# HannesStark/3DInfomax

Hardware: AMD Instinct MI355X
Metric: molecules/sec pretraining step (PNA+Net3D, QM9-50k); PNA-agg HBM GB/s vs peak (higher is better)
Workload: dtype f32

## Files before the change

### 3dinfomax_amd/net3d_native.py

```python
import ctypes
import os

import torch

from . import _lib, ops, tape
from .layer_native import _Arena, _al, _tail
from .layers import _composite_ok, _keeps_pre, _set_workspaces

NATIVE_NET3D = True
BF16_STORE = True
BF16_STORE_MIN_EDGES = 1 << 20
FUSED_EDGE = True
_F32 = torch.float32


def _chk(rc, name):
    if rc != 0:
        _lib.check(rc, name)


def _blocks(model):
    b = model.__dict__.get('_i3d_blocks')
    if b is None:
        layers = [(list(l.message_network.fully_connected), l.soft_edge_network, list(l.update_network.fully_connected), l.reduce_mean)
                  for l in model.mp_layers]
        nw = list(model.node_wise_output_network.fully_connected) if model.node_wise_output_layers > 0 else []
        b = model.__dict__['_i3d_blocks'] = (model.edge_input.fully_connected[0], layers, nw, list(model.output.fully_connected))
    return b


def eligible(model, g):
    if not (NATIVE_NET3D and model.training and not model.use_node_features):
        return False
    idx = g.index()
    if g.device.type != 'cuda' or idx.num_edges == 0 or idx.num_graphs == 0:
        return False
    edge_in, layers, nw, out = _blocks(model)
    fcs = [edge_in] + [fc for m, _, u, _ in layers for fc in m + u] + nw + out[:-1]
    for fc in fcs:
        h = fc.hot()
        if not (_composite_ok(h[4]) and h[0].is_cuda and h[0].is_contiguous() and h[1] is not None and fc.bias):
            return False
    last = out[-1].hot()
    if last[4].bn is not None:
        if not (_composite_ok(last[4]) and last[0].is_contiguous()):
            return False
    elif last[4].act is not None or not last[0].is_contiguous() or last[1] is None:
        return False
    return len(layers) >= 1 and all(len(m) >= 1 and len(u) >= 1 for m, _, u, _ in layers)


def fused_edge_ok(model):
    ok = model.__dict__.get('_i3d_fused_edge')
    if ok is None:
        edge_in, layers, nw, out = _blocks(model)
        ok = False
        if len(layers) == 1 and len(layers[0][0]) == 1:
            H = model.node_embedding.shape[0]
            w_in, spec_in = edge_in.hot('silu')[0], edge_in.hot('silu')[4]
            w_m, spec_m = layers[0][0][0].hot()[0], layers[0][0][0].hot()[4]
            n_enc = model.fourier_encodings
            din = 2 * n_enc + 1 if n_enc > 0 else 1
            ok = (tuple(w_in.shape) == (H, din) and tuple(w_m.shape) == (H, 3 * H) and spec_in.act == 'silu'
                  and spec_m.act == 'silu' and spec_m.post_act is None
                  and bool(_lib.load().i3d_net3d_edge_supported(H, n_enc)))
        model.__dict__['_i3d_fused_edge'] = ok
    return ok and FUSED_EDGE


def _edge_stage_fwd(L, stream, ar, dev, model, g, idx, d_raw, edge_in, msg_fc, se, reduce_mean, N, E, H):
    a = _lib.Net3dEdgeArgs()
    W_in, b_in, g_in, be_in, spec_in = edge_in.hot('silu')[:5]
    W_m, b_m, g_m, be_m, spec_m = msg_fc.hot()[:5]
    _tail(a.tail_in, spec_in, g_in, be_in, ar.take(H), ar.take(H), H, dev)
    _tail(a.tail_msg, spec_m, g_m, be_m, ar.take(H), ar.take(H), H, dev)
    a.num_nodes, a.num_edges, a.hidden, a.n_enc, a.reduce_mean = N, E, H, model.fourier_encodings, int(reduce_mean)
    a.ld_w_in, a.ld_w_msg = W_in.stride(0), W_m.stride(0)
    a.d_raw, a.perm, a.dst_s, a.in_ptr = d_raw.data_ptr(), idx.perm.data_ptr(), idx.dst_s.data_ptr(), idx.in_ptr.data_ptr()
    a.emb = model.node_embedding.data_ptr()
    a.W_in, a.b_in, a.W_msg, a.b_msg = W_in.data_ptr(), b_in.data_ptr(), W_m.data_ptr(), b_m.data_ptr()
    a.w_gate, a.b_gate = se.weight.data_ptr(), se.bias.data_ptr()
    a.stats = ar.take(int(L.i3d_net3d_edge_stats_floats(E, H)))
    a.aff_in, a.aff_msg = ar.take(3 * H), ar.take(3 * H)
    a.x_msg, a.msg, a.m_sum = ar.take(E * H), ar.take(E * H), ar.take(N * H)
    d_out = torch.empty(E, H, dtype=_F32, device=dev)
    a.d_out = d_out.data_ptr()
    a.store_bf16 = int(BF16_STORE and E >= BF16_STORE_MIN_EDGES and L.i3d_get_matmul_precision() != 0)
    a.x_center = ar.take(H)
    _chk(L.i3d_net3d_edge_fwd(ctypes.byref(a), stream), 'i3d_net3d_edge_fwd')
    return a, a.m_sum, d_out, (W_in, b_in, g_in, be_in, W_m, b_m, g_m, be_m, se.weight, se.bias)


class _Rec:
    __slots__ = ('kind', 'a', 'fc', 'rows', 'fin', 'fout', 'x', 'y', 'extra')

    def __init__(self, kind, **kw):
        self.a = self.fc = self.extra = None
        self.rows = self.fin = self.fout = self.x = self.y = 0
        self.kind = kind
        for k, v in kw.items():
            setattr(self, k, v)


def _fc_floats(rows, fout, spec):
    return _al(rows * fout) * (3 if _keeps_pre(spec) else 2) + 2 * _al(fout)


def _fc_fwd(L, stream, ar, dev, fc, rows, x_ptr, residual=None, post_act=None, y_ptr=None):
    W, b, gamma, beta, spec = fc.hot(post_act)[:5]
    fout, fin = W.shape
    a = _lib.FcArgs()
    _tail(a.tail, spec, gamma, beta, ar.take(fout), ar.take(fout), fout, dev)
    a.rows, a.f_in, a.f_out, a.ldw = rows, fin, fout, W.stride(0)
    a.x, a.W, a.bias, a.residual = x_ptr, W.data_ptr(), b.data_ptr(), residual
    a.xact = ar.take(rows * fout)
    a.pre_keep = ar.take(rows * fout) if _keeps_pre(spec) else None
    a.y = y_ptr if y_ptr is not None else ar.take(rows * fout)
    _chk(L.i3d_fc_bn_fwd(ctypes.byref(a), stream), 'i3d_fc_bn_fwd')
    return _Rec('fc', a=a, fc=fc, rows=rows, fin=fin, fout=fout, x=x_ptr, y=a.y, extra=(W, b, gamma, beta, residual is not None))


def forward(ctx, model, g, params):
    idx = g.index()
    dev = g.device
    N, E, B = idx.num_nodes, idx.num_edges, idx.num_graphs
    edge_in, layers, nw, out = _blocks(model)
    H = model.node_embedding.shape[0]
    n_enc = model.fourier_encodings
    enc_dim = 2 * n_enc + 1 if n_enc > 0 else 1
    codes = model._readout_codes
    R = len(codes)
    L = _lib.load()
    stream = ops._stream()

    fused = fused_edge_ok(model)
    total = _al(N * H)
    if fused:
        total += 5 * _al(H) + 2 * _al(3 * H) + _al(int(L.i3d_net3d_edge_stats_floats(E, H))) + 2 * _al(E * H) + 2 * _al(N * H)
    else:
        total += _al(E) + (_al(E * enc_dim) if n_enc > 0 else 0) + _fc_floats(E, H, edge_in.hot('silu')[4])
    for msg, se, upd, _ in layers:
        if not fused:
            Fo = msg[0].hot()[0].shape[0]
            total += _al(N * 2 * Fo) + _al(E * Fo) + _fc_floats(E, Fo, msg[0].hot()[4])
            for fc in msg[1:]:
                total += _fc_floats(E, fc.hot()[0].shape[0], fc.hot()[4])
            total += _al(E * H) * 2 + _al(E) + _al(N * H) * 2
        for fc in upd:
            total += _fc_floats(N, fc.hot()[0].shape[0], fc.hot()[4])
    for fc in nw:
        total += _fc_floats(N, fc.hot()[0].shape[0], fc.hot()[4])
    total += _al(B * R * H)
    for fc in out:
        total += _fc_floats(B, fc.hot()[0].shape[0], fc.hot()[4]) if fc.hot()[4].bn is not None else 0
    ar = _Arena(total + 64, dev)
    tr = {'layers': [], 'nw': [], 'out': []}

    d_raw = g.edata['d']
    if d_raw.dtype != _F32 or not d_raw.is_contiguous():
        d_raw = d_raw.contiguous().float()
    emb = model.node_embedding
    h = ar.take(N * H)
    _chk(L.i3d_broadcast_row(emb.data_ptr(), N, H, h, stream), 'i3d_broadcast_row')
    d_out = d = None
    if not fused:
        dperm = ar.take(E)
        _chk(L.i3d_gather_rows(d_raw.data_ptr(), idx.perm.data_ptr(), E, 1, dperm, stream), 'i3d_gather_rows')
        enc = dperm
        if n_enc > 0:
            enc = ar.take(E * enc_dim)
            _chk(L.i3d_fourier_encode(dperm, E, n_enc, enc, stream), 'i3d_fourier_encode')
        tr['edge_in'] = _fc_fwd(L, stream, ar, dev, edge_in, E, enc, post_act='silu')
        d = tr['edge_in'].y

    last_h_fc = nw[-1] if nw else layers[-1][2][-1]
    h_out = torch.empty(N, last_h_fc.hot()[0].shape[0], dtype=_F32, device=dev)
    n_layers = len(layers)
    for li, (msg, se, upd, reduce_mean) in enumerate(layers):
        last_layer = li + 1 == n_layers
        lay = {'msg': [], 'upd': []}
        if fused:
            lay['fused'], m_sum, d_out, ctx.fused_params = _edge_stage_fwd(L, stream, ar, dev, model, g, idx, d_raw, edge_in,
                                                                           msg[0], se, reduce_mean, N, E, H)
            u = ar.take(N * H)
            _chk(L.i3d_add(m_sum, h, N * H, u, stream), 'i3d_add')
            x = u
            for k, fc in enumerate(upd):
                final = k + 1 == len(upd)
                y_ptr = h_out.data_ptr() if (final and not nw) else None
                r = _fc_fwd(L, stream, ar, dev, fc, N, x, residual=h if final else None, y_ptr=y_ptr)
                lay['upd'].append(r)
                x = r.y
            tr['layers'].append(lay)
            h = x
            break
        W, b, gamma, beta, spec = msg[0].hot()[:5]
        Fo = W.shape[0]
        a = _lib.EdgeFcArgs()
        _tail(a.tail, spec, gamma, beta, ar.take(Fo), ar.take(Fo), Fo, dev)
        a.num_nodes, a.num_edges, a.f_h, a.f_q, a.f_out, a.ldw = N, E, H, H, Fo, W.stride(0)
        a.h, a.q, a.W, a.bias = h, d, W.data_ptr(), b.data_ptr()
        a.src_s, a.dst_s, a.in_ptr = idx.src_s.data_ptr(), idx.dst_s.data_ptr(), idx.in_ptr.data_ptr()
        a.out_ptr, a.out_epos = idx.out_ptr.data_ptr(), idx.out_epos.data_ptr()
        a.P, a.Q = ar.take(N * 2 * Fo), ar.take(E * Fo)
        a.xact = ar.take(E * Fo)
        a.pre_keep = ar.take(E * Fo) if _keeps_pre(spec) else None
        a.y = ar.take(E * Fo)
        _chk(L.i3d_edge_fc_bn_fwd(ctypes.byref(a), stream), 'i3d_edge_fc_bn_fwd')
        lay['edge'] = _Rec('edge', a=a, fc=msg[0], fout=Fo, x=h, y=a.y, extra=(W, b, gamma, beta))
        m = a.y
        for fc in msg[1:]:
            r = _fc_fwd(L, stream, ar, dev, fc, E, m)
            lay['msg'].append(r)
            m = r.y
        d_next = d
        if not last_layer:
            d_next = ar.take(E * H)
            _chk(L.i3d_add(d, m, E * H, d_next, stream), 'i3d_add')
        msg_w, gate, m_sum, u = ar.take(E * H), ar.take(E), ar.take(N * H), ar.take(N * H)
        sw, sb = se.weight, se.bias
        _chk(L.i3d_soft_edge_fwd(m, sw.data_ptr(), sb.data_ptr(), E, H, msg_w, gate, stream), 'i3d_soft_edge_fwd')
        _chk(L.i3d_segment_sum(msg_w, H, idx.in_ptr.data_ptr(), None, N, H, int(reduce_mean), m_sum, H, stream), 'i3d_segment_sum')
        _chk(L.i3d_add(m_sum, h, N * H, u, stream), 'i3d_add')
        lay['gate'] = _Rec('gate', x=m, y=gate, extra=(sw, sb, reduce_mean))
        x = u
        for k, fc in enumerate(upd):
            final = k + 1 == len(upd)
            y_ptr = h_out.data_ptr() if (final and last_layer and not nw) else None
            r = _fc_fwd(L, stream, ar, dev, fc, N, x, residual=h if final else None, y_ptr=y_ptr)
            lay['upd'].append(r)
            x = r.y
        tr['layers'].append(lay)
        h, d = x, d_next
    for k, fc in enumerate(nw):
        r = _fc_fwd(L, stream, ar, dev, fc, N, h, y_ptr=h_out.data_ptr() if k + 1 == len(nw) else None)
        tr['nw'].append(r)
        h = r.y
    g.ndata['feat'] = h_out
    if d_out is None:
        d_out = torch.empty(E, H, dtype=_F32, device=dev)
        _chk(L.i3d_gather_rows(d, idx.inv_perm.data_ptr(), E, H, d_out.data_ptr(), stream), 'i3d_gather_rows')
    g.edata['d'] = d_out

    ro = ar.take(B * R * H)
    _chk(L.i3d_segment_readout_fwd(h, idx.graph_ptr.data_ptr(), B, H, _lib.int_array(codes), R, ro, stream), 'i3d_segment_readout_fwd')
    tr['readout'] = _Rec('readout', x=h, y=ro)
    x, fin = ro, R * H
    z = None
    for k, fc in enumerate(out):
        W, b, gamma, beta, spec = fc.hot()[:5]
        final = k + 1 == len(out)
        if final:
            z = torch.empty(B, W.shape[0], dtype=_F32, device=dev)
        if spec.bn is not None:
            r = _fc_fwd(L, stream, ar, dev, fc, B, x, y_ptr=z.data_ptr() if final else None)
            x, fin = r.y, W.shape[0]
        else:
            _chk(L.i3d_gemm_f32(0, 1, B, W.shape[0], fin, x, fin, W.data_ptr(), W.stride(0), z.data_ptr(), W.shape[0], b.data_ptr(), 0,
                                stream), 'i3d_gemm_f32')
            r = _Rec('linear', rows=B, fin=fin, fout=W.shape[0], x=x, extra=(W, b))
        tr['out'].append(r)
    ctx.native = (ar, tr, idx, emb, (N, E, B, H), codes, h_out, (d_raw, d_out) if fused else None)
    ctx.params = params
    return z


def _fc_bwd(L, stream, ar, dev, r, grad_y, grads, need_x=True):
    a = r.a
    W, b, gamma, beta, _ = r.extra
    a.grad_y = grad_y
    a.grad_pre = ar.take(r.rows * r.fout)
    gW, gb, gg, gbe = tape.grad_like(W), tape.grad_like(b), tape.grad_like(gamma), tape.grad_like(beta)
    grads[id(W)], grads[id(b)], grads[id(gamma)], grads[id(beta)] = gW, gb, gg, gbe
    a.grad_W, a.grad_bias, a.grad_gamma, a.grad_beta = gW.data_ptr(), gb.data_ptr(), gg.data_ptr(), gbe.data_ptr()
    a.grad_x = ar.take(r.rows * r.fin) if need_x else None
    _set_workspaces(a.tail, r.fout, dev)
    _chk(L.i3d_fc_bn_bwd(ctypes.byref(a), stream), 'i3d_fc_bn_bwd')
    return a.grad_x


def _edge_stage_bwd(L, stream, ar, dev, a, gu, gh_l, emb, grads, ctx, N, E, H, ws_h):
    model_params = ctx.fused_params
    bufs = [tape.grad_like(t) for t in model_params]
    for t, b in zip(model_params, bufs):
        grads[id(t)] = b
    (a.grad_W_in, a.grad_b_in, a.grad_gamma_in, a.grad_beta_in, a.grad_W_msg, a.grad_b_msg, a.grad_gamma_msg, a.grad_beta_msg,
     a.grad_w_gate, a.grad_b_gate) = [b.data_ptr() for b in bufs]
    gemb = tape.grad_like(emb)
    grads[id(emb)] = gemb
    _chk(L.i3d_colsum(gh_l, None, N, H, gemb.data_ptr(), ws_h, stream), 'i3d_colsum')
    a.grad_emb = gemb.data_ptr()
    a.grad_m_sum = gu
    a.grad_ya, a.grad_lin = ar.take(E * H), None
    a.partial = ar.take(int(L.i3d_net3d_edge_bwd_floats(E, H, a.n_enc)))
    _chk(L.i3d_net3d_edge_bwd(ctypes.byref(a), stream), 'i3d_net3d_edge_bwd')


def _bwd_floats(tr, N, E, H, L):
    def fc(r):
        return _al(r.rows * r.fout) + _al(r.rows * r.fin)
    total = 64 + _al(N * H)
    if 'edge_in' in tr:
        total += fc(tr['edge_in'])
    for r in tr['out']:
        total += fc(r) if r.kind == 'fc' else _al(r.rows * r.fin)
    for r in tr['nw']:
        total += fc(r)
    for lay in tr['layers']:
        total += sum(fc(r) for r in lay['upd'] + lay['msg'])
        if 'fused' in lay:
            a = lay['fused']
            total += _al(N * H) + _al(E * H) + _al(int(L.i3d_net3d_edge_bwd_floats(E, H, a.n_enc)))
            continue
        Fo = lay['edge'].fout
        total += 2 * _al(N * H) + 3 * _al(E * H) + _al(E) + _al(E * Fo) + _al(N * 2 * Fo)
    return total


def backward(ctx, grad_z):
    ar_f, tr, idx, emb, (N, E, B, H), codes, h_out, _edge_keep = ctx.native
    dev = grad_z.device
    grad_z = grad_z.contiguous()
    L = _lib.load()
    stream = ops._stream()
    grads = {}
    ar = _Arena(_bwd_floats(tr, N, E, H, L), dev)
    ws_h = ops._workspace(H, dev).data_ptr()

    g = grad_z.data_ptr()
    for r in reversed(tr['out']):
        if r.kind == 'linear':
            W, b = r.extra
            gW, gb = tape.grad_like(W), tape.grad_like(b)
            grads[id(W)], grads[id(b)] = gW, gb
            _chk(L.i3d_gemm_f32_ws(1, 0, r.fout, r.fin, r.rows, g, r.fout, r.x, r.fin, gW.data_ptr(), W.stride(0), None, 0,
                                   ops._gemm_workspace(dev).data_ptr(), ops.GEMM_WORKSPACE_BYTES, stream), 'i3d_gemm_f32_ws')
            _chk(L.i3d_colsum(g, None, r.rows, r.fout, gb.data_ptr(), ops._workspace(r.fout, dev).data_ptr(), stream), 'i3d_colsum')
            gx = ar.take(r.rows * r.fin)
            _chk(L.i3d_gemm_f32(0, 0, r.rows, r.fin, r.fout, g, r.fout, W.data_ptr(), W.stride(0), gx, r.fin, None, 0, stream),
                 'i3d_gemm_f32')
            g = gx
        else:
            g = _fc_bwd(L, stream, ar, dev, r, g, grads)
    gh = ar.take(N * H)
    _chk(L.i3d_segment_readout_bwd(g, tr['readout'].x, idx.graph_ptr.data_ptr(), B, H, _lib.int_array(codes), len(codes), gh, stream),
         'i3d_segment_readout_bwd')
    for r in reversed(tr['nw']):
        gh = _fc_bwd(L, stream, ar, dev, r, gh, grads)
    gd = None
    for lay in reversed(tr['layers']):
        gu = gh
        for r in reversed(lay['upd']):
            gu = _fc_bwd(L, stream, ar, dev, r, gu, grads)
        if 'fused' in lay:
            gh_l = ar.take(N * H)
            _chk(L.i3d_add(gh, gu, N * H, gh_l, stream), 'i3d_add')
            _edge_stage_bwd(L, stream, ar, dev, lay['fused'], gu, gh_l, emb, grads, ctx, N, E, H, ws_h)
            return tuple(grads.get(id(p)) for p in ctx.params)
        gate = lay['gate']
        sw, sb, reduce_mean = gate.extra
        gh_l = ar.take(N * H)
        _chk(L.i3d_add(gh, gu, N * H, gh_l, stream), 'i3d_add')
        gmsg = ar.take(E * H)
        _chk(L.i3d_segment_bcast(gu, idx.in_ptr.data_ptr(), idx.dst_s.data_ptr(), E, H, int(reduce_mean), gmsg, stream),
             'i3d_segment_bcast')
        gm, gg = ar.take(E * H), ar.take(E)
        _chk(L.i3d_soft_edge_bwd(gmsg, gate.x, gate.y, sw.data_ptr(), E, H, gm, gg, stream), 'i3d_soft_edge_bwd')
        gsw, gsb = tape.grad_like(sw), tape.grad_like(sb)
        grads[id(sw)], grads[id(sb)] = gsw, gsb
        _chk(L.i3d_colsum(gate.x, gg, E, H, gsw.data_ptr(), ws_h, stream), 'i3d_colsum')
        _chk(L.i3d_colsum(gg, None, E, 1, gsb.data_ptr(), ops._workspace(1, dev).data_ptr(), stream), 'i3d_colsum')
        if gd is not None:
            _chk(L.i3d_add_inplace(gm, gd, E * H, stream), 'i3d_add_inplace')
        for r in reversed(lay['msg']):
            gm = _fc_bwd(L, stream, ar, dev, r, gm, grads)
        e = lay['edge']
        a = e.a
        W, b, gamma, beta = e.extra
        Fo = e.fout
        a.grad_y, a.grad_pre, a.grad_P = gm, ar.take(E * Fo), ar.take(N * 2 * Fo)
        gW, gb, gga, gbe = tape.grad_like(W), tape.grad_like(b), tape.grad_like(gamma), tape.grad_like(beta)
        grads[id(W)], grads[id(b)], grads[id(gamma)], grads[id(beta)] = gW, gb, gga, gbe
        a.grad_W, a.grad_bias, a.grad_gamma, a.grad_beta = gW.data_ptr(), gb.data_ptr(), gga.data_ptr(), gbe.data_ptr()
        a.grad_h, a.grad_q = ar.take(N * H), ar.take(E * H)
        _set_workspaces(a.tail, Fo, dev)
        _chk(L.i3d_edge_fc_bn_bwd(ctypes.byref(a), stream), 'i3d_edge_fc_bn_bwd')
        _chk(L.i3d_add_inplace(gh_l, a.grad_h, N * H, stream), 'i3d_add_inplace')
        if gd is not None:
            _chk(L.i3d_add_inplace(a.grad_q, gd, E * H, stream), 'i3d_add_inplace')
        gd, gh = a.grad_q, gh_l
    _fc_bwd(L, stream, ar, dev, tr['edge_in'], gd, grads, need_x=False)
    gemb = tape.grad_like(emb)
    grads[id(emb)] = gemb
    _chk(L.i3d_colsum(gh, None, N, H, gemb.data_ptr(), ws_h, stream), 'i3d_colsum')
    return tuple(grads.get(id(p)) for p in ctx.params)
```

### include/infomax3d_hip.h

```cpp
#ifndef INFOMAX3D_HIP_H
#define INFOMAX3D_HIP_H

#include <stdint.h>

#ifdef __cplusplus
extern "C" {
#endif

#define I3D_OK 0
#define I3D_ERR_INVALID (-1)
#define I3D_ERR_LAUNCH (-2)
#define I3D_NOT_TAKEN 1

#define I3D_ACT_NONE 0
#define I3D_ACT_RELU 1
#define I3D_ACT_SILU 2
#define I3D_ACT_SIGMOID 3
#define I3D_ACT_LEAKY_RELU 4
#define I3D_ACT_TANH 5
#define I3D_ACT_ELU 6
#define I3D_ACT_SELU 7
#define I3D_ACT_SOFTPLUS 8

#define I3D_AGG_MEAN 0
// ... 458 lines not shown
    void* Wcat_panel;
    void* Wcat_dgrad_panel;
} I3dPnaLayerArgs;

typedef struct {
    const float* running_mean;
    const float* running_var;
    const float* gamma;
    const float* beta;
    float* aff;
    int feat;
    float eps;
} I3dBnEvalAff;
int i3d_bn_eval_aff_multi(const I3dBnEvalAff* entries , int n, void* stream);

long i3d_pna_layer_stats_floats(int num_nodes, int num_edges, int m_padded, int f);

typedef struct {
    I3dBnTail tail_in;
    I3dBnTail tail_msg;
    int num_nodes, num_edges, hidden, n_enc, reduce_mean;
    int ld_w_in, ld_w_msg;
    const float* d_raw;
    const int* perm;
    const int* dst_s;
    const int* in_ptr;
    const float* emb;
    const float* W_in;
    const float* b_in;
    const float* W_msg;
    const float* b_msg;
    const float* w_gate;
    const float* b_gate;
    float* stats;
    float* aff_in;
    float* aff_msg;
    float* x_msg;
    float* d_out;
    float* msg;
    float* m_sum;
    const float* grad_m_sum;
    float* grad_ya;
    float* grad_lin;
    float* partial;
    float* grad_W_in;
    float* grad_b_in;
    float* grad_gamma_in;
    float* grad_beta_in;
    float* grad_W_msg;
    float* grad_b_msg;
    float* grad_gamma_msg;
    float* grad_beta_msg;
    float* grad_w_gate;
    float* grad_b_gate;
    float* grad_emb;
    int store_bf16;
    float* x_center;
} I3dNet3dEdgeArgs;
int i3d_net3d_edge_supported(int hidden, int n_enc);
long i3d_net3d_edge_stats_floats(int num_edges, int hidden);
long i3d_net3d_edge_bwd_floats(int num_edges, int hidden, int n_enc);
int i3d_net3d_edge_fwd(const I3dNet3dEdgeArgs* args, void* stream);
int i3d_net3d_edge_bwd(const I3dNet3dEdgeArgs* args, void* stream);

int i3d_event_create(void** event);
int i3d_event_destroy(void* event);
int i3d_event_record(void* event, void* stream);
int i3d_event_elapsed_ms(void* start, void* stop, float* ms);

int i3d_wgrad_stream_join(void* stream);
int i3d_wgrad_stream_fork(void* stream, void** side);
int i3d_wgrad_stream_peek(void* stream, void** side);
int i3d_pna_layer_weights_fwd(const I3dPnaLayerArgs* args, void* stream);
int i3d_pna_layer_fwd(const I3dPnaLayerArgs* args, void* stream);
int i3d_pna_layer_bwd(const I3dPnaLayerArgs* args, void* stream);
int i3d_fc_bn_fwd(const I3dFcArgs* args, void* stream);
int i3d_fc_bn_bwd(const I3dFcArgs* args, void* stream);
int i3d_fc_bn_bwd_chain(const I3dFcArgs* args, void* stream);
int i3d_fc_bn_bwd_wgrad(const I3dFcArgs* args, void* stream);
int i3d_edge_fc_bn_fwd(const I3dEdgeFcArgs* args, void* stream);
int i3d_edge_fc_bn_bwd(const I3dEdgeFcArgs* args, void* stream);
int i3d_grouped_fc_bn_fwd(const I3dGroupedFcArgs* args, void* stream);
int i3d_grouped_fc_bn_bwd(const I3dGroupedFcArgs* args, void* stream);

#define I3D_MAX_LAYERS 16
#define I3D_MAX_HEAD_FC 4
typedef struct {
    const float* W;
    const float* bias;
    const float* gamma;
    const float* beta;
    float* running_mean;
    float* running_var;
    long long* num_batches_tracked;
    float* grad_W;
    float* grad_bias;
    float* grad_gamma;
    float* grad_beta;
    int f_in, f_out, act;
    float eps, momentum;
} I3dFcParams;

typedef struct {
    int training;
    int n_layers, hidden, n_pre, residual;
    int n_aggregators, aggregators[8];
    int n_scalers, scalers[4];
    float avg_d_log;
    I3dFcParams pre[I3D_MAX_LAYERS][I3D_MAX_EXTRA_FC + 1];
    I3dFcParams post[I3D_MAX_LAYERS];
    int n_atom_tables, atom_dims[16];
    const float* atom_tables[16];
    float* grad_atom_tables;
    int n_bond_tables, bond_dims[16];
    const float* bond_tables[16];
    float* grad_bond_tables;
    int n_readout, readout_ops[4];
    int n_head;
    I3dFcParams head[I3D_MAX_HEAD_FC];
} I3dPnaModel;

typedef struct {
    int num_nodes, num_edges, num_graphs;
    const int64_t* atom_feat;
    const int64_t* bond_feat;
    const int* in_ptr;
    const int* perm;
    const int* src_s;
    const int* dst_s;
    const int* out_ptr;
    const int* out_epos;
    const int* graph_ptr;
    const int* deg_rows;
    const int* deg_tile_group;
    int m_padded, n_groups;
    int group_degree[32], group_start[32], group_count[32];
    const int64_t* comb;
    int n_comb, v_pad;
} I3dPnaBatch;

long i3d_pna_model_saved_floats(const I3dPnaModel* model, const I3dPnaBatch* batch);
long i3d_pna_model_scratch_floats(const I3dPnaModel* model, const I3dPnaBatch* batch);
int i3d_pna_model_fwd(const I3dPnaModel* model, const I3dPnaBatch* batch, float* saved, float* node_emb, float* edge_emb,
                      float* out, void* bn_workspace, void* const* agg_events, void* stream, void** ctx_out);
int i3d_pna_model_bwd(void* ctx, const I3dPnaModel* grads_from, const float* grad_out, float* scratch, void* bn_workspace,
                      void* gemm_workspace, long gemm_workspace_bytes, void* stream);
int i3d_pna_model_bwd_part(void* ctx, const I3dPnaModel* grads_from, const float* grad_out, float* scratch, void* bn_workspace,
                           void* gemm_workspace, long gemm_workspace_bytes, int part, int split, void* stream);
int i3d_pna_model_ctx_free(void* ctx);
int i3d_pna_messages_normalized(const float* e, const float* aff, long rows, int feat, float* out, void* stream);
int i3d_pna_messages_normalized_ex(const void* e, int e_bf16, const float* aff, long rows, int feat, float* out, void* stream);
int i3d_pna_model_debug_messages(void* ctx, int layer, float* out, void* stream);

int i3d_adam_chunk_elems(void);
int i3d_adam_chunk_bytes(void);
int i3d_adam_step(const void* chunk_table, int n_chunks, float* steps, int n_steps, double lr, double beta1, double beta2,
                  double weight_decay, double eps, double bias_correction1, double bias_correction2_sqrt, void* stream);

int i3d_ema_chunk_elems(void);
int i3d_ema_chunk_bytes(void);
int i3d_ema_update(const void* chunk_table, int n_chunks, float decay, float one_minus_decay, void* stream);

long i3d_contrastive_metrics_out_doubles(int D1, int D2);
long i3d_contrastive_metrics_work_floats(int B1, int B2, int D1, int D2, int pairwise);
int i3d_contrastive_metrics(const float* z1, const float* z2, int B1, int B2, int D1, int D2, int pairwise, float threshold, float t,
                            float alpha, float* work, double* out, void* stream);

int i3d_complete_graph_build(const float* coords, const int* graph_ptr, const int* edge_ptr, int num_graphs,
                             int num_nodes, int num_edges, int* in_ptr, int* src_s, int* dst_s, int* perm,
                             int* inv_perm, int* out_epos, int64_t* src_id, int64_t* dst_id, float* d_id,
                             void* stream);

int i3d_mha_fwd(const float* qkv, const int* graph_ptr, int num_graphs, int num_nodes, int hidden, int nhead, float scale,
                float* out, float* lse, void* stream);
int i3d_mha_bwd(const float* qkv, const float* out, const float* grad_out, const float* lse, const int* graph_ptr,
                int num_graphs, int num_nodes, int hidden, int nhead, float scale, float* delta, float* grad_qkv,
                void* stream);
int i3d_ln_res_fwd(const float* x, const float* r, const float* gamma, const float* beta, int rows, int feat, float eps,
                   float* y, float* mean, float* rstd, void* stream);
long i3d_ln_res_partial_floats(int rows, int feat);
int i3d_ln_res_bwd(const float* grad_y, const float* x, const float* r, const float* gamma, const float* mean,
                   const float* rstd, int rows, int feat, float* grad_x, float* partial, float* grad_gamma, float* grad_beta,
                   void* stream);
int i3d_pair_sum_fwd(const float* u, const float* bias, const int* src_s, const int* dst_s, const int* perm, int pairs,
                     int feat, float* out, void* stream);
int i3d_pair_sum_bwd(const float* grad_out, const float* u, const float* bias, const int* src_s, const int* dst_s,
                     const int* perm, int pairs, int feat, float* grad_pair, void* stream);
int i3d_pair_norm_fwd(const float* p, const int* src_s, const int* dst_s, const int* perm, int pairs, int feat, float* out,
                      void* stream);
int i3d_pair_norm_bwd(const float* grad_out, const float* p, const float* dist, const int* src_s, const int* dst_s,
                      const int* perm, int pairs, int feat, float* grad_pair, void* stream);

typedef struct {
    const unsigned char* keep;
    const int* graph_ptr;
    const int* edge_ptr;
    const int* deg_base;
    const int* pad_range;
    int n_groups, num_nodes, num_edges, rows;
    int64_t *src, *dst, *atom_feat, *bond_feat;
    int *in_ptr, *perm, *src_s, *dst_s, *out_ptr, *out_epos, *inv_perm, *deg_rows;
} I3dNodeDropView;
int i3d_node_drop_build(const int64_t* src, const int64_t* dst, const int64_t* atom_feat, const int64_t* bond_feat,
                        const int* in_ptr, const int* perm, const int* src_s, const int* dst_s, const int* out_ptr,
                        const int* out_epos, const int* graph_ptr, int num_graphs, int atom_cols, int bond_cols,
                        int max_atoms, int max_edges, int deg_stride, const I3dNodeDropView* views, int n_views,
                        void* stream);

#define I3D_NOISED_DISTANCES 0
#define I3D_NOISED_COORDINATES 1
int i3d_noised_graph_build(const float* coords, const int* graph_ptr, const int* edge_ptr, int num_graphs, int num_nodes,
                           int num_edges, int num_noised, int mode, float std_, unsigned long long seed,
                           unsigned long long step, int* in_ptr, int* src_s, int* dst_s, int* perm, int* inv_perm,
                           int* out_epos, int* graph_ptr_out, int64_t* src_id, int64_t* dst_id, float* d_id, float* x_out,
                           void* stream);

int i3d_pair_mlp_supported(int width);
long i3d_pair_mlp_workspace_floats(int pairs, int width);
int i3d_pair_mlp_fwd(const float* AB, const float* b1, const float* gamma, const float* beta, const float* w2, const float* b2,
                     const int* src_s, const int* dst_s, const int* perm, int pairs, int width, int training, float eps,
                     float momentum, float* running_mean, float* running_var, int64_t* num_batches_tracked, double* stats,
                     double* coef, float* workspace, float* out, void* stream);
int i3d_pair_mlp_bwd(const float* grad_out, const double* coef, const float* AB, const float* b1, const float* gamma,
                     const float* beta, const float* w2, const int* src_s, const int* dst_s, const int* perm, const int* in_ptr,
                     const int* out_ptr, const int* out_epos, int num_nodes, int pairs, int width, int training,
                     const double* stats, float* workspace, float* grad_pair, double* bcoef, float* grad_AB, float* grad_gamma,
                     float* grad_beta, float* grad_w2, float* grad_b2, void* stream);
long i3d_mse_partial_floats(long n);
int i3d_mse_fwd(const float* a, const float* b, long n, double scale, float* partial, float* loss, void* stream);
int i3d_mse_bwd(const float* a, const float* b, long n, double scale, const float* grad_scale, float* grad_a, float* grad_b,
                void* stream);

int i3d_row_normalize_fwd(const float* x, int rows, int dim, float* y, float* norms, void* stream);
int i3d_row_normalize_bwd(const float* x, const float* norms, const float* grad_y, int rows, int dim, float* grad_x, void* stream);
int i3d_sep2d_max_conformers(void);
int i3d_sep2d_fwd(const float* sim, const float* n1, const float* n2, int batch, int conf, float tau, double* row_den,
                  double* row_pos, float* loss, void* stream);
int i3d_sep2d_bwd(const float* sim, const float* n1, const float* n2, const double* row_den, const double* row_pos, int batch,
                  int conf, float tau, const float* grad_scale, float* dsim, float* ca, float* cb, void* stream);
int i3d_mmd_pair_fwd(const float* X, const float* Y, int batch, int conf, int dim, int kernel_num, double kernel_mul, float* cross,
                     float* intra, float* bandwidth, float* sim, void* stream);
int i3d_mmd_pair_bwd(const float* X, const float* Y, const float* cross, const float* intra, const float* bandwidth,
                     const float* sim, const float* dsim, int batch, int conf, int dim, int kernel_num, double kernel_mul,
                     float* gcross, float* gintra, float* dX, float* dY, void* stream);

int i3d_kl_mp_fwd(const float* z1, const float* z2, int batch, int conf, int dim, double inv_global_batch, double* stats, float* loss,
                  void* stream);
int i3d_kl_mp_bwd(const float* z1, const float* z2, int batch, int conf, int dim, double inv_global_batch, const float* grad_scale,
                  float* dz1, float* dz2, void* stream);

int i3d_gauss_lik_fwd(const float* z1, const float* z2, int batch, int conf, int dim, long mol_stride, long conf_stride, double* lik,
                      void* stream);
int i3d_gauss_lik_loss(const double* lik, int batch, double tau, double* rows, float* loss, void* stream);
int i3d_gauss_lik_probs(const double* lik, int batch, double* out, void* stream);
int i3d_gauss_lik_bwd(const float* z1, const float* z2, int batch, int conf, int dim, long mol_stride, long conf_stride,
                      const double* lik, const double* rows, double tau, const float* grad_scale, double* grad_lik, float* dz1,
                      float* dz2, void* stream);
int i3d_gauss_jsd_fwd(const float* z1, const float* z2, int batch, int conf, int dim, double* astat, double* sim, double* rows,
                      float* loss, void* stream);
int i3d_gauss_jsd_bwd(const float* z1, const float* z2, int batch, int conf, int dim, const double* astat, const double* rows,
                      const float* grad_scale, float* dz1, float* dz2, void* stream);

long i3d_masked_loss_partial_floats(int rows, int tasks);
int i3d_masked_loss_fwd(const float* pred, const float* target, int rows, int tasks, int kind, float* partials, double* out,
                        void* stream);
int i3d_masked_loss_bwd(const float* pred, const float* target, int rows, int tasks, int kind, const double* out,
                        const float* grad_out, float* grad_pred, void* stream);
long i3d_task_moments_partial_floats(int rows, int tasks);
int i3d_task_moments(const float* pred, const float* target, int rows, int tasks, float* partials, double* table, void* stream);

int i3d_gin_chunk_edges(void);
long i3d_gin_conv_bwd_partial_floats(int num_nodes, int num_edges, int feat, int num_codes);
int i3d_gin_conv_fwd(const float* h, const float* vn, const int* graph_ptr, int num_graphs, const float* T, int num_codes,
                     const int* codes, const int* in_ptr, const int* src_s, const float* eps, int num_nodes, int num_edges, int feat,
                     float* x, float* z, void* stream);
int i3d_gin_conv_bwd(const float* g, const float* x, const float* T, int num_codes, const int* codes, const int* src_s,
                     const int* dst_s, const int* out_ptr, const int* out_epos, const int* code_order, const int* code_ptr,
                     const float* eps, int num_nodes, int num_edges, int feat, float* partials, float* dx, float* dT, float* deps,
                     void* stream);

int i3d_gate_reduce_max_feat(void);
int i3d_gate_reduce_fwd(const float* m, const float* ws, const float* bs, const int* in_ptr, const float* h, int num_nodes,
                        int num_edges, int feat, int reduce_mean, float* u, float* w, void* stream);
int i3d_gate_reduce_bwd(const float* gu, const float* m, const float* w, const float* ws, const int* in_ptr, int num_nodes,
                        int num_edges, int feat, int reduce_mean, float* gm, float* part_ws, float* part_bs, void* stream);

#define I3D_GEOMOL_PARTIAL_FLOATS 2048
int i3d_geomol_edge_fwd(const float* F, const float* PQ, const int* src_s, const int* dst_s, int num_nodes, int num_edges, int feat,
                        float* h, void* stream);
int i3d_geomol_edge_bwd(const float* g, const float* h, const int* in_ptr, const int* out_ptr, const int* out_epos, int num_nodes,
                        int num_edges, int feat, float* dF, float* dPQ, void* stream);
int i3d_geomol_residual_fwd(const float* a, const float* b, const float* eps, long rows, int feat, float* out, void* stream);
int i3d_geomol_residual_bwd(const float* g, const float* a, const float* eps, long rows, int feat, float* partials, float* da,
                            float* deps, void* stream);

int i3d_lg_row_chunk(void);
long i3d_lg_ntxent_scratch_floats(int n, int b);
long i3d_lg_ntxent_work_floats(int n, int b, int dim);
int i3d_lg_ntxent_fwd(const float* zn, const float* zg, const int* graph_ptr, int n, int b, int dim, float tau, float eps,
                      int norm, float* scratch, float* loss, void* stream);
int i3d_lg_ntxent_bwd(const float* zn, const float* zg, const int* graph_ptr, int n, int b, int dim, float tau, float eps,
                      int norm, const float* scratch, const float* grad_scale_dev, float* work, float* dzn, float* dzg,
                      void* stream);

int i3d_conf_match_max_conformers(void);
int i3d_per_conf_max_conformers(void);
// ... 89 lines not shown
```

Measured before the change: 272,400.

## Move Net3D forward/backward launch sequencing into a native C++ sequencer

Adds a C++ entry point that plans buffer layouts and issues the full Net3D forward and backward kernel sequence (edge stage, FC+BN blocks, readout, output layers) in single native calls. The Python side caches the parameter and gradient descriptor structs and the per-batch sizes, replacing many per-layer ctypes calls and Python bookkeeping. This is meant to cut host launch overhead in a step made of many small kernels, at the cost of a second code path that must stay in sync with the Python one.

New measurement: 269,500. -1.1%, worse.

```diff
diff --git a/3dinfomax_amd/csrc/net3d_model.hip b/3dinfomax_amd/csrc/net3d_model.hip
--- /dev/null
+++ b/3dinfomax_amd/csrc/net3d_model.hip
@@ -0,0 +1,341 @@
+#include "common.h"
+
+#include <new>
+#include <vector>
+
+using namespace i3d;
+
+#define TRY(call)                 \
+    do {                          \
+        int rc_ = (call);         \
+        if (rc_ != I3D_OK) return rc_; \
+    } while (0)
+
+namespace {
+
+inline long al4(long n) { return (n + 3) & ~3L; }
+
+struct Bump {
+    float* base;
+    long used = 0;
+    explicit Bump(float* b) : base(b) {}
+    float* take(long n) {
+        float* p = base ? base + used : nullptr;
+        used += al4(n);
+        return p;
+    }
+};
+
+struct Net3dCtx {
+    I3dNet3dEdgeArgs edge;
+    std::vector<I3dFcParams> p;
+    std::vector<I3dFcArgs> fc;
+    int n_update = 0, n_node_wise = 0, n_out = 0, n_readout = 0;
+    int readout_ops[8];
+    int N = 0, E = 0, B = 0, H = 0;
+    const int* graph_ptr = nullptr;
+    float* h0 = nullptr;
+    float* u = nullptr;
+    float* h_last = nullptr;
+    float* readout = nullptr;
+    const float* lin_x = nullptr;
+    float* z = nullptr;
+    int f_node = 0;
+};
+
+void set_ws(I3dBnTail& t, void* bn_ws, void* gemm_ws, long gemm_ws_bytes) {
+    t.workspace = bn_ws;
+    t.gemm_workspace = gemm_ws;
+    t.gemm_workspace_bytes = gemm_ws_bytes;
+}
+
+inline bool keeps_pre(int act) { return !(act == I3D_ACT_NONE || act == I3D_ACT_RELU || act == I3D_ACT_LEAKY_RELU); }
+
+int check_desc(const I3dNet3dEdgeArgs* e, const I3dFcParams* blocks, int n_update, int n_node_wise, int n_out, int n_readout,
+               const I3dPnaBatch* b) {
+    I3D_CHECK_ARG(e != nullptr && blocks != nullptr && b != nullptr, "null description");
+    I3D_CHECK_ARG(n_update >= 1 && n_node_wise >= 0 && n_out >= 1 && n_readout >= 1 && n_readout <= 8, "block / readout counts");
+    I3D_CHECK_ARG(b->num_nodes > 0 && b->num_edges > 0 && b->num_graphs > 0, "empty batch");
+    I3D_CHECK_ARG(e->hidden > 0 && i3d_net3d_edge_supported(e->hidden, e->n_enc), "hidden width / Fourier order without an edge kernel");
+    const int n = n_update + n_node_wise + n_out;
+    int f = e->hidden;
+    for (int i = 0; i < n; ++i) {
+        const I3dFcParams& p = blocks[i];
+        if (i == n_update + n_node_wise) f *= n_readout;
+        I3D_CHECK_ARG(p.f_in == f && p.f_out > 0, "block widths do not chain");
+        I3D_CHECK_ARG(p.gamma != nullptr || (i == n - 1 && p.act == I3D_ACT_NONE), "a block without BatchNorm that is not the last Linear");
+        f = p.f_out;
+    }
+    I3D_CHECK_ARG(blocks[n_update - 1].f_out == e->hidden, "the residual of the last update block needs f_out == hidden");
+    return I3D_OK;
+}
+
+void plan_fc(Bump& ar, I3dFcArgs& a, const I3dFcParams& p, int rows, const float* x, const float* residual, bool y_given,
+             float* y) {
+    a = I3dFcArgs{};
+    a.tail.act = p.act;
+    a.tail.post_act = I3D_ACT_NONE;
+    a.tail.eps = p.eps;
+    a.tail.momentum = p.momentum;
+    a.tail.gamma = p.gamma;
+    a.tail.beta = p.beta;
+    a.tail.running_mean = p.running_mean;
+    a.tail.running_var = p.running_var;
+    a.tail.num_batches_tracked = p.num_batches_tracked;
+    a.tail.mean = ar.take(p.f_out);
+    a.tail.invstd = ar.take(p.f_out);
+    a.rows = rows;
+    a.f_in = p.f_in;
+    a.f_out = p.f_out;
+    a.ldw = p.f_in;
+    a.x = x;
+    a.W = p.W;
+    a.bias = p.bias;
+    a.residual = residual;
+    a.xact = ar.take((long)rows * p.f_out);
+    a.pre_keep = keeps_pre(p.act) ? ar.take((long)rows * p.f_out) : nullptr;
+    a.y = y_given ? y : ar.take((long)rows * p.f_out);
+}
+
+long plan_forward(Net3dCtx& c, float* saved, float* node_emb_out, float* d_out, float* z_out) {
+    Bump ar(saved);
+    const long N = c.N, E = c.E, B = c.B, H = c.H;
+    I3dNet3dEdgeArgs& e = c.edge;
+    c.h0 = ar.take(N * H);
+    e.tail_in.mean = ar.take(H);
+    e.tail_in.invstd = ar.take(H);
+    e.tail_msg.mean = ar.take(H);
+    e.tail_msg.invstd = ar.take(H);
+    e.stats = ar.take(i3d_net3d_edge_stats_floats(c.E, c.H));
+    e.aff_in = ar.take(3 * H);
+    e.aff_msg = ar.take(3 * H);
+    e.x_msg = ar.take(E * H);
+    e.msg = ar.take(E * H);
+    e.m_sum = ar.take(N * H);
+    e.d_out = d_out;
+    e.x_center = ar.take(H);
+    c.u = ar.take(N * H);
+    const int n_node = c.n_update + c.n_node_wise;
+    c.fc.assign(c.p.size(), I3dFcArgs{});
+    const float* x = c.u;
+    for (int i = 0; i < n_node; ++i) {
+        const bool last = i + 1 == n_node;
+        plan_fc(ar, c.fc[i], c.p[i], c.N, x, i + 1 == c.n_update ? c.h0 : nullptr, last, node_emb_out);
+        x = c.fc[i].y;
+    }
+    c.h_last = node_emb_out;
+    c.f_node = c.p[n_node - 1].f_out;
+    c.readout = ar.take(B * c.n_readout * c.f_node);
+    x = c.readout;
+    c.lin_x = nullptr;
+    for (int i = n_node; i < n_node + c.n_out; ++i) {
+        const bool last = i + 1 == n_node + c.n_out;
+        if (c.p[i].gamma != nullptr) {
+            plan_fc(ar, c.fc[i], c.p[i], c.B, x, nullptr, last, z_out);
+            x = c.fc[i].y;
+        } else {
+            c.lin_x = x;
+        }
+    }
+    c.z = z_out;
+    return ar.used + 64;
+}
+
+struct BwdPlan {
+    std::vector<float*> grad_pre, grad_x;
+    float* gh = nullptr;
+    float* gh_l = nullptr;
+    float* grad_ya = nullptr;
+    float* partial = nullptr;
+    long used = 0;
+};
+
+void plan_backward(const Net3dCtx& c, float* scratch, BwdPlan& bp) {
+    Bump ar(scratch);
+    const long N = c.N, E = c.E, H = c.H;
+    const int n_node = c.n_update + c.n_node_wise, n = n_node + c.n_out;
+    bp.grad_pre.assign(n, nullptr);
+    bp.grad_x.assign(n, nullptr);
+    for (int i = n - 1; i >= n_node; --i) {
+        const I3dFcParams& p = c.p[i];
+        if (p.gamma != nullptr) bp.grad_pre[i] = ar.take((long)c.B * p.f_out);
+        bp.grad_x[i] = ar.take((long)c.B * p.f_in);
+    }
+    bp.gh = ar.take(N * c.f_node);
+    for (int i = n_node - 1; i >= 0; --i) {
+        const I3dFcParams& p = c.p[i];
+        bp.grad_pre[i] = ar.take(N * p.f_out);
+        bp.grad_x[i] = ar.take(N * p.f_in);
+    }
+    bp.gh_l = ar.take(N * H);
+    bp.grad_ya = ar.take(E * H);
+    bp.partial = ar.take(i3d_net3d_edge_bwd_floats(c.E, c.H, c.edge.n_enc));
+    bp.used = ar.used + 64;
+}
+
+int fill_ctx(Net3dCtx& c, const I3dNet3dEdgeArgs* e, const I3dFcParams* blocks, int n_update, int n_node_wise, int n_out,
+             const int* readout_ops, int n_readout, const I3dPnaBatch* b, const float* d_raw) {
+    c.edge = *e;
+    c.p.assign(blocks, blocks + n_update + n_node_wise + n_out);
+    c.n_update = n_update;
+    c.n_node_wise = n_node_wise;
+    c.n_out = n_out;
+    c.n_readout = n_readout;
+    for (int k = 0; k < n_readout; ++k) c.readout_ops[k] = readout_ops ? readout_ops[k] : 0;
+    c.N = b->num_nodes;
+    c.E = b->num_edges;
+    c.B = b->num_graphs;
+    c.H = e->hidden;
+    c.graph_ptr = b->graph_ptr;
+    c.edge.num_nodes = c.N;
+    c.edge.num_edges = c.E;
+    c.edge.d_raw = d_raw;
+    c.edge.perm = b->perm;
+    c.edge.dst_s = b->dst_s;
+    c.edge.in_ptr = b->in_ptr;
+    c.edge.grad_m_sum = nullptr;
+    c.edge.grad_ya = c.edge.grad_lin = c.edge.partial = nullptr;
+    return I3D_OK;
+}
+
+}
+
+extern "C" long i3d_net3d_model_saved_floats(const I3dNet3dEdgeArgs* edge, const I3dFcParams* blocks, int n_update, int n_node_wise,
+                                             int n_out, int n_readout, const I3dPnaBatch* batch) {
+    if (check_desc(edge, blocks, n_update, n_node_wise, n_out, n_readout, batch) != I3D_OK) return -1;
+    Net3dCtx c;
+    fill_ctx(c, edge, blocks, n_update, n_node_wise, n_out, nullptr, n_readout, batch, nullptr);
+    return plan_forward(c, nullptr, nullptr, nullptr, nullptr);
+}
+
+extern "C" long i3d_net3d_model_scratch_floats(const I3dNet3dEdgeArgs* edge, const I3dFcParams* blocks, int n_update, int n_node_wise,
+                                               int n_out, int n_readout, const I3dPnaBatch* batch) {
+    if (check_desc(edge, blocks, n_update, n_node_wise, n_out, n_readout, batch) != I3D_OK) return -1;
+    Net3dCtx c;
+    fill_ctx(c, edge, blocks, n_update, n_node_wise, n_out, nullptr, n_readout, batch, nullptr);
+    plan_forward(c, nullptr, nullptr, nullptr, nullptr);
+    BwdPlan bp;
+    plan_backward(c, nullptr, bp);
+    return bp.used;
+}
+
+extern "C" int i3d_net3d_model_fwd(const I3dNet3dEdgeArgs* edge, const I3dFcParams* blocks, int n_update, int n_node_wise, int n_out,
+                                   const int* readout_ops, int n_readout, const I3dPnaBatch* batch, const float* d_raw, float* saved,
+                                   long saved_floats, float* node_emb_out, float* d_out, float* z_out, void* bn_workspace, void* stream,
+                                   void** ctx_out) {
+    I3D_CHECK_ARG(ctx_out != nullptr, "null ctx_out");
+    *ctx_out = nullptr;
+    TRY(check_desc(edge, blocks, n_update, n_node_wise, n_out, n_readout, batch));
+    I3D_CHECK_ARG(readout_ops != nullptr && d_raw != nullptr && saved != nullptr && node_emb_out != nullptr && d_out != nullptr &&
+                      z_out != nullptr && bn_workspace != nullptr, "null buffer");
+    I3D_CHECK_ARG(batch->perm != nullptr && batch->dst_s != nullptr && batch->in_ptr != nullptr && batch->graph_ptr != nullptr,
+                  "null index");
+    I3D_CHECK_ARG(edge->emb != nullptr && edge->W_in != nullptr && edge->b_in != nullptr && edge->W_msg != nullptr &&
+                      edge->b_msg != nullptr && edge->w_gate != nullptr && edge->b_gate != nullptr && edge->tail_in.gamma != nullptr &&
+                      edge->tail_msg.gamma != nullptr, "null parameter");
+    for (int i = 0; i < n_update + n_node_wise + n_out; ++i)
+        I3D_CHECK_ARG(blocks[i].W != nullptr && blocks[i].bias != nullptr, "null parameter");
+    Net3dCtx* c = new (std::nothrow) Net3dCtx();
+    I3D_CHECK_ARG(c != nullptr, "out of host memory");
+    fill_ctx(*c, edge, blocks, n_update, n_node_wise, n_out, readout_ops, n_readout, batch, d_raw);
+    const long need = plan_forward(*c, saved, node_emb_out, d_out, z_out);
+    if (saved_floats < need) {
+        delete c;
+        I3D_CHECK_ARG(false, "saved buffer smaller than i3d_net3d_model_saved_floats");
+    }
+    *ctx_out = c;
+    const long N = c->N, H = c->H;
+    const int n_node = n_update + n_node_wise, n = n_node + n_out;
+    TRY(i3d_broadcast_row(c->edge.emb, N, c->H, c->h0, stream));
+    set_ws(c->edge.tail_in, bn_workspace, nullptr, 0);
+    set_ws(c->edge.tail_msg, bn_workspace, nullptr, 0);
+    TRY(i3d_net3d_edge_fwd(&c->edge, stream));
+    TRY(i3d_add(c->edge.m_sum, c->h0, N * H, c->u, stream));
+    for (int i = 0; i < n_node; ++i) {
+        set_ws(c->fc[i].tail, bn_workspace, nullptr, 0);
+        TRY(i3d_fc_bn_fwd(&c->fc[i], stream));
+    }
+    TRY(i3d_segment_readout_fwd(c->h_last, c->graph_ptr, c->B, c->f_node, c->readout_ops, n_readout, c->readout, stream));
+    for (int i = n_node; i < n; ++i) {
+        const I3dFcParams& p = c->p[i];
+        if (p.gamma != nullptr) {
+            set_ws(c->fc[i].tail, bn_workspace, nullptr, 0);
+            TRY(i3d_fc_bn_fwd(&c->fc[i], stream));
+        } else {
+            TRY(i3d_gemm_f32(0, 1, c->B, p.f_out, p.f_in, c->lin_x, p.f_in, p.W, p.f_in, z_out, p.f_out, p.bias, 0, stream));
+        }
+    }
+    return I3D_OK;
+}
+
+extern "C" int i3d_net3d_model_bwd(void* ctx, const I3dNet3dEdgeArgs* ge, const I3dFcParams* gb, const float* grad_z, float* scratch,
+                                   long scratch_floats, void* bn_workspace, void* gemm_workspace, long gemm_workspace_bytes,
+                                   void* stream) {
+    I3D_CHECK_ARG(ctx != nullptr && ge != nullptr && gb != nullptr && grad_z != nullptr && scratch != nullptr && bn_workspace != nullptr,
+                  "null");
+    Net3dCtx* c = static_cast<Net3dCtx*>(ctx);
+    const int n_node = c->n_update + c->n_node_wise, n = n_node + c->n_out;
+    I3D_CHECK_ARG(ge->grad_W_in && ge->grad_b_in && ge->grad_gamma_in && ge->grad_beta_in && ge->grad_W_msg && ge->grad_b_msg &&
+                      ge->grad_gamma_msg && ge->grad_beta_msg && ge->grad_w_gate && ge->grad_b_gate && ge->grad_emb,
+                  "gradient buffers of the edge stage not set");
+    for (int i = 0; i < n; ++i)
+        I3D_CHECK_ARG(gb[i].grad_W != nullptr && gb[i].grad_bias != nullptr &&
+                          (c->p[i].gamma == nullptr || (gb[i].grad_gamma != nullptr && gb[i].grad_beta != nullptr)),
+                      "gradient buffers of a block not set");
+    BwdPlan bp;
+    plan_backward(*c, scratch, bp);
+    I3D_CHECK_ARG(scratch_floats >= bp.used, "scratch smaller than i3d_net3d_model_scratch_floats");
+    const long N = c->N, H = c->H;
+    const float* g = grad_z;
+    for (int i = n - 1; i >= 0; --i) {
+        const I3dFcParams& p = c->p[i];
+        if (i == n_node - 1) {
+            TRY(i3d_segment_readout_bwd(g, c->h_last, c->graph_ptr, c->B, c->f_node, c->readout_ops, c->n_readout, bp.gh, stream));
+            g = bp.gh;
+        }
+        if (p.gamma == nullptr) {
+            TRY(i3d_gemm_f32_ws(1, 0, p.f_out, p.f_in, c->B, g, p.f_out, c->lin_x, p.f_in, gb[i].grad_W, p.f_in, nullptr, 0,
+                                gemm_workspace, gemm_workspace_bytes, stream));
+            TRY(i3d_colsum(g, nullptr, c->B, p.f_out, gb[i].grad_bias, bn_workspace, stream));
+            TRY(i3d_gemm_f32(0, 0, c->B, p.f_in, p.f_out, g, p.f_out, p.W, p.f_in, bp.grad_x[i], p.f_in, nullptr, 0, stream));
+        } else {
+            I3dFcArgs& a = c->fc[i];
+            a.grad_y = g;
+            a.grad_pre = bp.grad_pre[i];
+            a.grad_W = gb[i].grad_W;
+            a.grad_bias = gb[i].grad_bias;
+            a.grad_gamma = gb[i].grad_gamma;
+            a.grad_beta = gb[i].grad_beta;
+            a.grad_x = bp.grad_x[i];
+            set_ws(a.tail, bn_workspace, gemm_workspace, gemm_workspace_bytes);
+            TRY(i3d_fc_bn_bwd(&a, stream));
+        }
+        g = bp.grad_x[i];
+    }
+    const float* gh_res = c->fc[c->n_update - 1].grad_y;
+    const float* gu = g;
+    TRY(i3d_add(gh_res, gu, N * H, bp.gh_l, stream));
+    I3dNet3dEdgeArgs& e = c->edge;
+    e.grad_W_in = ge->grad_W_in;
+    e.grad_b_in = ge->grad_b_in;
+    e.grad_gamma_in = ge->grad_gamma_in;
+    e.grad_beta_in = ge->grad_beta_in;
+    e.grad_W_msg = ge->grad_W_msg;
+    e.grad_b_msg = ge->grad_b_msg;
+    e.grad_gamma_msg = ge->grad_gamma_msg;
+    e.grad_beta_msg = ge->grad_beta_msg;
+    e.grad_w_gate = ge->grad_w_gate;
+    e.grad_b_gate = ge->grad_b_gate;
+    e.grad_emb = ge->grad_emb;
+    TRY(i3d_colsum(bp.gh_l, nullptr, c->N, c->H, e.grad_emb, bn_workspace, stream));
+    e.grad_m_sum = gu;
+    e.grad_ya = bp.grad_ya;
+    e.grad_lin = nullptr;
+    e.partial = bp.partial;
+    return i3d_net3d_edge_bwd(&e, stream);
+}
+
+extern "C" int i3d_net3d_model_ctx_free(void* ctx) {
+    delete static_cast<Net3dCtx*>(ctx);
+    return I3D_OK;
+}
diff --git a/3dinfomax_amd/net3d_native.py b/3dinfomax_amd/net3d_native.py
--- a/3dinfomax_amd/net3d_native.py
+++ b/3dinfomax_amd/net3d_native.py
@@ -1,5 +1,5 @@
 import ctypes
-import os
+import itertools
 
 import torch
 
@@ -11,6 +11,7 @@
 BF16_STORE = True
 BF16_STORE_MIN_EDGES = 1 << 20
 FUSED_EDGE = True
+C_SEQUENCER = True
 _F32 = torch.float32
 
 
@@ -120,7 +121,182 @@
     return _Rec('fc', a=a, fc=fc, rows=rows, fin=fin, fout=fout, x=x_ptr, y=a.y, extra=(W, b, gamma, beta, residual is not None))
 
 
+
+_serial = itertools.count(1)
+
+
+class _Desc:
+    __slots__ = ('edge', 'blocks', 'counts', 'codes', 'n_codes', 'key', 'keep', 'bn_feat', 'f_node', 'target_dim', 'hidden',
+                 'plist', 'ret_idx', 'serial')
+
+
+def _tail_desc(tail, spec, gamma, beta):
+    bn = spec.bn
+    tail.act, tail.post_act = ops.ACT[spec.act], ops.ACT[spec.post_act]
+    tail.eps, tail.momentum = bn.eps, bn.momentum
+    tail.gamma, tail.beta = gamma.data_ptr(), beta.data_ptr()
+    tail.running_mean, tail.running_var = bn.running_mean.data_ptr(), bn.running_var.data_ptr()
+    nbt = bn.num_batches_tracked
+    tail.num_batches_tracked = nbt.data_ptr() if nbt is not None else None
+    return [gamma, beta, bn.running_mean, bn.running_var, nbt]
+
+
+def _describe(model, params):
+    edge_in, layers, nw, out = _blocks(model)
+    msg, se, upd, reduce_mean = layers[0]
+    W_in, b_in, g_in, be_in, spec_in = edge_in.hot('silu')[:5]
+    W_m, b_m, g_m, be_m, spec_m = msg[0].hot()[:5]
+    emb = model.node_embedding
+    H = emb.shape[0]
+    d = _Desc()
+    e = d.edge = _lib.Net3dEdgeArgs()
+    keep = _tail_desc(e.tail_in, spec_in, g_in, be_in) + _tail_desc(e.tail_msg, spec_m, g_m, be_m)
+    e.hidden, e.n_enc, e.reduce_mean = H, model.fourier_encodings, int(reduce_mean)
+    e.ld_w_in, e.ld_w_msg = W_in.stride(0), W_m.stride(0)
+    e.emb = emb.data_ptr()
+    e.W_in, e.b_in, e.W_msg, e.b_msg = W_in.data_ptr(), b_in.data_ptr(), W_m.data_ptr(), b_m.data_ptr()
+    e.w_gate, e.b_gate = se.weight.data_ptr(), se.bias.data_ptr()
+    plist = [W_in, b_in, g_in, be_in, W_m, b_m, g_m, be_m, se.weight, se.bias, emb]
+    fcs = upd + nw + out
+    blocks = d.blocks = (_lib.FcParams * len(fcs))()
+    bn_feat = H
+    for dst, fc in zip(blocks, fcs):
+        W, b, gamma, beta, spec = fc.hot()[:5]
+        dst.W, dst.bias = W.data_ptr(), b.data_ptr()
+        dst.f_out, dst.f_in = W.shape
+        dst.act = ops.ACT[spec.act]
+        plist += [W, b]
+        if spec.bn is not None:
+            bn = spec.bn
+            dst.gamma, dst.beta = gamma.data_ptr(), beta.data_ptr()
+            dst.running_mean, dst.running_var = bn.running_mean.data_ptr(), bn.running_var.data_ptr()
+            nbt = bn.num_batches_tracked
+            dst.num_batches_tracked = nbt.data_ptr() if nbt is not None else None
+            dst.eps, dst.momentum = bn.eps, bn.momentum
+            keep += [bn.running_mean, bn.running_var, nbt]
+            plist += [gamma, beta]
+        bn_feat = max(bn_feat, W.shape[0])
+    codes = model._readout_codes
+    d.counts = (len(upd), len(nw), len(out))
+    d.codes, d.n_codes = _lib.int_array(codes), len(codes)
+    d.keep, d.plist, d.bn_feat, d.hidden = keep, plist, bn_feat, H
+    d.f_node = (nw[-1] if nw else upd[-1]).hot()[0].shape[0]
+    d.target_dim = out[-1].hot()[0].shape[0]
+    pos = {id(p): i for i, p in enumerate(plist)}
+    d.ret_idx = [pos.get(id(p), -1) for p in params]
+    d.serial = next(_serial)
+    return d
+
+
+def _describe_grads(desc, bufs):
+    d = _Desc()
+    e = d.edge = _lib.Net3dEdgeArgs()
+    ptr = [b.data_ptr() for b in bufs]
+    (e.grad_W_in, e.grad_b_in, e.grad_gamma_in, e.grad_beta_in, e.grad_W_msg, e.grad_b_msg, e.grad_gamma_msg, e.grad_beta_msg,
+     e.grad_w_gate, e.grad_b_gate, e.grad_emb) = ptr[:11]
+    k = 11
+    blocks = d.blocks = (_lib.FcParams * len(desc.blocks))()
+    for dst, src in zip(blocks, desc.blocks):
+        dst.grad_W, dst.grad_bias = ptr[k], ptr[k + 1]
+        k += 2
+        if src.gamma:
+            dst.grad_gamma, dst.grad_beta = ptr[k], ptr[k + 1]
+            k += 2
+    d.key, d.serial = tuple(ptr), desc.serial
+    return d
+
+
+def _batch_struct(idx, desc):
+    st = idx.__dict__.get('_i3d_net3d_batch')
+    if st is None:
+        b = _lib.PnaBatch()
+        b.num_nodes, b.num_edges, b.num_graphs = idx.num_nodes, idx.num_edges, idx.num_graphs
+        b.in_ptr, b.perm, b.dst_s, b.graph_ptr = idx.in_ptr.data_ptr(), idx.perm.data_ptr(), idx.dst_s.data_ptr(), idx.graph_ptr.data_ptr()
+        st = idx.__dict__['_i3d_net3d_batch'] = [b, 0, 0, 0]
+    if st[1] != desc.serial:
+        L = _lib.load()
+        nu, nn, no = desc.counts
+        args = (ctypes.byref(desc.edge), desc.blocks, nu, nn, no, desc.n_codes, ctypes.byref(st[0]))
+        n_saved, n_scratch = L.i3d_net3d_model_saved_floats(*args), L.i3d_net3d_model_scratch_floats(*args)
+        if n_saved < 0 or n_scratch < 0:
+            _lib.check(_lib.DEFINES['I3D_ERR_INVALID'], 'i3d_net3d_model_saved_floats')
+        st[1], st[2], st[3] = desc.serial, n_saved, n_scratch
+    return st[0], st[2], st[3]
+
+
+class _CtxHandle:
+
+    def __init__(self, ptr):
+        self.ptr = ptr
+
+    def __del__(self):
+        try:
+            if self.ptr:
+                _lib.load().i3d_net3d_model_ctx_free(self.ptr)
+        except Exception:
+            pass
+
+
+def _forward_c(ctx, model, g, params):
+    idx = g.index()
+    dev = g.device
+    desc = model.__dict__.get('_i3d_n3_desc_fwd')
+    key = (tuple([id(p) for p in params]), tuple([p.data_ptr() for p in params]))
+    if desc is None or desc.key != key:
+        desc = _describe(model, params)
+        desc.key = key
+        model.__dict__['_i3d_n3_desc_fwd'] = desc
+    b, n_saved, n_scratch = _batch_struct(idx, desc)
+    d_raw = g.edata['d']
+    if d_raw.dtype != _F32 or not d_raw.is_contiguous():
+        d_raw = d_raw.contiguous().float()
+    L = _lib.load()
+    N, E, B = idx.num_nodes, idx.num_edges, idx.num_graphs
+    e = desc.edge
+    e.store_bf16 = int(BF16_STORE and E >= BF16_STORE_MIN_EDGES and L.i3d_get_matmul_precision() != 0)
+    saved = torch.empty(n_saved, dtype=_F32, device=dev)
+    h_out = torch.empty(N, desc.f_node, dtype=_F32, device=dev)
+    d_out = torch.empty(E, desc.hidden, dtype=_F32, device=dev)
+    z = torch.empty(B, desc.target_dim, dtype=_F32, device=dev)
+    nu, nn, no = desc.counts
+    handle = ctypes.c_void_p()
+    rc = L.i3d_net3d_model_fwd(ctypes.byref(e), desc.blocks, nu, nn, no, desc.codes, desc.n_codes, ctypes.byref(b), d_raw.data_ptr(),
+                               saved.data_ptr(), n_saved, h_out.data_ptr(), d_out.data_ptr(), z.data_ptr(),
+                               ops._workspace(desc.bn_feat, dev).data_ptr(), ops._stream(), ctypes.byref(handle))
+    holder = _CtxHandle(handle.value)
+    _chk(rc, 'i3d_net3d_model_fwd')
+    g.ndata['feat'] = h_out
+    g.edata['d'] = d_out
+    ctx.native_c = (holder, model, desc, n_scratch, (saved, idx, d_raw, d_out, h_out))
+    ctx.params = params
+    return z
+
+
+def _backward_c(ctx, grad_z):
+    st = ctx.native_c
+    if st is None:
+        raise RuntimeError('Net3D: trying to backward through the network a second time: its saved activations were freed by '
+                           'the first backward pass')
+    holder, model, desc, n_scratch, _keep = st
+    dev = grad_z.device
+    grad_z = grad_z.contiguous()
+    bufs = [tape.grad_like(p) for p in desc.plist]
+    gd = model.__dict__.get('_i3d_n3_desc_bwd')
+    if gd is None or gd.serial != desc.serial or gd.key != tuple([t.data_ptr() for t in bufs]):
+        gd = model.__dict__['_i3d_n3_desc_bwd'] = _describe_grads(desc, bufs)
+    scratch = torch.empty(n_scratch, dtype=_F32, device=dev)
+    L = _lib.load()
+    _chk(L.i3d_net3d_model_bwd(holder.ptr, ctypes.byref(gd.edge), gd.blocks, grad_z.data_ptr(), scratch.data_ptr(), n_scratch,
+                               ops._workspace(desc.bn_feat, dev).data_ptr(), ops._gemm_workspace(dev).data_ptr(),
+                               ops.GEMM_WORKSPACE_BYTES, ops._stream()), 'i3d_net3d_model_bwd')
+    ctx.native_c = None
+    return tuple([bufs[i] if i >= 0 else None for i in desc.ret_idx])
+
+
 def forward(ctx, model, g, params):
+    if C_SEQUENCER and fused_edge_ok(model):
+        return _forward_c(ctx, model, g, params)
+    ctx.native_c = False
     idx = g.index()
     dev = g.device
     N, E, B = idx.num_nodes, idx.num_edges, idx.num_graphs
@@ -318,6 +494,8 @@
 
 
 def backward(ctx, grad_z):
+    if ctx.native_c is not False:
+        return _backward_c(ctx, grad_z)
     ar_f, tr, idx, emb, (N, E, B, H), codes, h_out, _edge_keep = ctx.native
     dev = grad_z.device
     grad_z = grad_z.contiguous()
diff --git a/include/infomax3d_hip.h b/include/infomax3d_hip.h
--- a/include/infomax3d_hip.h
+++ b/include/infomax3d_hip.h
@@ -634,6 +634,19 @@
 int i3d_pna_messages_normalized_ex(const void* e, int e_bf16, const float* aff, long rows, int feat, float* out, void* stream);
 int i3d_pna_model_debug_messages(void* ctx, int layer, float* out, void* stream);
 
+long i3d_net3d_model_saved_floats(const I3dNet3dEdgeArgs* edge, const I3dFcParams* blocks, int n_update, int n_node_wise, int n_out,
+                                  int n_readout, const I3dPnaBatch* batch);
+long i3d_net3d_model_scratch_floats(const I3dNet3dEdgeArgs* edge, const I3dFcParams* blocks, int n_update, int n_node_wise, int n_out,
+                                    int n_readout, const I3dPnaBatch* batch);
+int i3d_net3d_model_fwd(const I3dNet3dEdgeArgs* edge, const I3dFcParams* blocks, int n_update, int n_node_wise, int n_out,
+                        const int* readout_ops, int n_readout, const I3dPnaBatch* batch, const float* d_raw, float* saved,
+                        long saved_floats, float* node_emb_out, float* d_out, float* z_out, void* bn_workspace, void* stream,
+                        void** ctx_out);
+int i3d_net3d_model_bwd(void* ctx, const I3dNet3dEdgeArgs* grads_edge, const I3dFcParams* grads_blocks, const float* grad_z,
+                        float* scratch, long scratch_floats, void* bn_workspace, void* gemm_workspace, long gemm_workspace_bytes,
+                        void* stream);
+int i3d_net3d_model_ctx_free(void* ctx);
+
 int i3d_adam_chunk_elems(void);
 int i3d_adam_chunk_bytes(void);
 int i3d_adam_step(const void* chunk_table, int n_chunks, float* steps, int n_steps, double lr, double beta1, double beta2,
```
